# ivargr/kmer_mapper

Hardware: AMD Instinct MI355X
Metric: M k-mers mapped/sec (whole node), k=31 150bp reads (higher is better)
Workload: dtype u64

## Files before the change

### kmer_mapper_amd/csrc/kmm.hip

```cpp
#include <hip/hip_runtime.h>

#include <climits>
#include <cstdarg>
#include <cstdint>
#include <cstdio>
#include <cstdlib>
#include <chrono>
#include <cstring>
#include <memory>
#include <mutex>
#include <string>
#include <thread>
#include <type_traits>
#include <utility>
#include <vector>

#include "kmm.h"
#include "kmm_radix_plan.hpp"

namespace {

thread_local std::string g_err;

int fail(int code, const char *fmt, ...)
// ... 253 lines not shown
    DevPtr<unsigned long long> stats;
    DevPtr<unsigned long long> queue;
    bool dynamic_schedule = true;
    int dyn_chunk = 16;
    uint64_t modulo = 0, magic = 0;
    int64_t n_entries = 0, max_node_id = 0;
    Stage stage[2];
    int cur = 0;
    int n_cu = 256;
    int path = 0;
    int grid_per_cu = 64;
    bool rx_ok = false;
    RxGeometry rx_geo;
    bool rx_no_mid = false;
    bool rx_flush_sorted = true;
    uint32_t rx_max_slice = 0;
    bool rx_fits_small = false, rx_fits_mid = false;
    int rx_grid_per_cu = 2;
    int64_t rx_min_units = 0;
    int64_t rx_sub_cap = RX_SUB_CAP_MAX;
    int64_t rx_sub_cap_eff = 0;
    int rx_sub_cap_eff_age = 0;
    int64_t rx_sub_cap_last = 0;
    const uint32_t *dbg_T1 = nullptr, *dbg_item_base = nullptr;
    const uint16_t *dbg_start1 = nullptr;
    uint32_t dbg_F1 = 0, dbg_NB = 0;
    int host_pack_threads = 0;
    std::unique_ptr<kmm_hostpack::Workers> pack_pool;
    PinnedBuf pack_pinned;
    PinnedBuf ring[RING_SLOTS];
    PinnedBuf pack_bits_pinned;
    int64_t host_packed_calls = 0, host_packed_record_calls = 0;
    int64_t host_pack_slice_kb = 0;
    DevBuf bgzf_comp[2], bgzf_raw[2], bgzf_meta[2], bgzf_tabs, bgzf_err, bgzf_carry, bgzf_crc, bgzf_status;
    Event bgzf_done[2];
    Event bgzf_slot_ev[RING_SLOTS];
    bool bgzf_used[2] = {false, false};
    int bgzf_cur = 0;
    int64_t bgzf_carry_len = 0;
    BgzfStaged bgzf_pre;
    bool bgzf_pre_valid = false;
    const uint8_t *bgzf_pre_from = nullptr, *bgzf_hint_ptr = nullptr;
    int64_t bgzf_pre_n = 0, bgzf_hint_n = 0;
    int bgzf_pre_buf = 0;
    int64_t bgzf_prestaged_calls = 0;
    int64_t bgzf_head_skip = 0;
    int64_t bgzf_tail_stop = -1;
    int64_t bgzf_calls = 0, bgzf_members = 0;
    DevBuf gz_comp, gz_raw, gz_carry, gz_window, gz_tabs, gz_meta, gz_res, gz_win, gz_gmaps, gz_gwin, gz_err;
    std::vector<DevBuf> gz_arena;
    kmm_gunzip::StreamState gz_state;
    int64_t gz_carry_len = 0;
    double gz_ratio = 4.0;
    int64_t gzip_calls = 0, gzip_members = 0, gzip_chunks = 0, gzip_false_starts = 0, gzip_continuations = 0, gzip_inflated = 0;
    int dbg_gzip_chunk_kb = 0;
    DevBuf bam_tiles[2], bam_bad, bam_base, bam_ctl, bam_out;
    int32_t bam_n_ref = -1;
    uint32_t bam_excl = 0;
    int64_t bam_calls = 0, bam_records = 0, bam_excluded = 0, bam_header_bytes = 0, bam_false_starts = 0, bam_continuations = 0;
    DevBuf rs_comp, rs_raw, rs_meta, rs_err, rs_status;
    int64_t bam_n_ref_param = -1;
    int64_t dbg_bam_resync_kb = 0;
    int64_t dbg_bgzf_call_cap_kb = 0;
    int64_t flat_uniform_batches = 0;
    DevBuf sam_tiles, sam_base, sam_ctl;
    int64_t sam_calls = 0, sam_records = 0, sam_excluded = 0, sam_header_lines = 0;
// ... 800 lines not shown
        if (bb >= 4) {
            ix->bloom_words = (uint32_t)(bb / 4);
            occ_bytes = (size_t)ix->bloom_words * 4;
        }
    }
    ix->occ_shift = occ_shift;
    ix->wide = !with_occ;
    if (const char *env = getenv("KMM_WIDE_BUCKETS"))
        ix->wide = atoi(env) != 0;
    HIPCHK(hipMalloc(ix->own_counts_buf.put(), sizeof(uint32_t) * (size_t)(ix->max_node_id + 1)));
    ix->counts = ix->own_counts_buf;
    HIPCHK(hipMemsetAsync(ix->counts, 0, sizeof(uint32_t) * (size_t)(ix->max_node_id + 1), ix->stream));
    HIPCHK(hipMalloc(ix->lut_default.put(), 256));
    HIPCHK(hipMalloc(ix->first_bad.put(), 3 * sizeof(unsigned long long)));
    HIPCHK(hipMalloc(ix->queue.put(), 4 * sizeof(unsigned long long)));
    HIPCHK(hipMalloc(ix->stats.put(), KMM_STAT_BYTES));
    HIPCHK(hipMemset(ix->stats, 0, KMM_STAT_BYTES));
    uint8_t lut[256];
    default_lut(lut);
    HIPCHK(hipMemcpy(ix->lut_default, lut, 256, hipMemcpyHostToDevice));
    HIPCHK(hipMalloc(ix->lut_codes.put(), 256));
    memset(lut, 0xFF, sizeof lut);
    lut[0] = 0; lut[1] = 1; lut[2] = 2; lut[3] = 3;
    HIPCHK(hipMemcpy(ix->lut_codes, lut, 256, hipMemcpyHostToDevice));
    unsigned long long nb[3] = {NO_BAD, NO_BAD, NO_BAD};
    HIPCHK(hipMemcpy(ix->first_bad, nb, sizeof nb, hipMemcpyHostToDevice));
    {
        const int budget = kmm_hostpack::cpu_budget();
        ix->host_pack_threads = budget >= 8 ? (budget < 16 ? budget : 16) : 0;
        if (const char *env = getenv("KMM_HOST_PACK_THREADS")) {
            const int v = atoi(env);
            ix->host_pack_threads = v < 0 ? 0 : (v > 256 ? 256 : v);
        }
    }

    if (ix->host_pack_threads > 0 && (size_t)(ix->max_node_id + 1) * 4 >= ((size_t)64 << 20))
        (void)ensure_ring(ix);

    DevBuf d_h2i, d_nk, d_km, d_nd, d_fr, d_err;
    bool staged = false;
    const int32_t *p_h2i = nullptr, *p_nk = nullptr, *p_nd = nullptr;
    const uint64_t *p_km = nullptr;
    const uint16_t *p_fr = nullptr;
    int rc = KMM_OK;
    do {
        if ((rc = stage_in<int32_t>(ix, d_h2i, h2i, (size_t)M, &p_h2i, &staged))) break;
        if ((rc = stage_in<int32_t>(ix, d_nk, nk, (size_t)M, &p_nk, &staged))) break;
        if ((rc = stage_in<uint64_t>(ix, d_km, kmers, (size_t)N, &p_km, &staged))) break;
        if ((rc = stage_in<int32_t>(ix, d_nd, nodes, (size_t)N, &p_nd, &staged))) break;
        if ((rc = stage_in<uint16_t>(ix, d_fr, freqs, (size_t)N, &p_fr, &staged))) break;
        if ((rc = ensure(d_err, 4))) break;
    } while (0);
    if (rc == KMM_OK) {
        hipError_t e = hipMemsetAsync(d_err.p, 0, 4, ix->copy_stream);
        if (e == hipSuccess) e = hipStreamSynchronize(ix->copy_stream);
        if (e != hipSuccess)
            rc = fail(KMM_ERR_HIP, "index upload: %s", hipGetErrorString(e));
    }
    uint32_t err = 0;
    if (rc == KMM_OK) {
        hipLaunchKernelGGL(k_validate_index, dim3(grid_for(ix, (int64_t)((M + 255) / 256), 16)), dim3(256), 0, ix->stream,
                           p_h2i, p_nk, p_nd, M, N, ix->max_node_id, (uint32_t *)d_err.p);
        hipError_t e = hipGetLastError();
        if (e == hipSuccess) e = hipStreamSynchronize(ix->stream);
        if (e == hipSuccess) e = hipMemcpy(&err, d_err.p, 4, hipMemcpyDeviceToHost);
        if (e != hipSuccess)
// ... 657 lines not shown
        KMMCHK(stage_copies_done(ix));
        HIPCHK(hipMemsetAsync(s.start_bits.p, 0, (size_t)n_words * 4, ix->stream));
        hipLaunchKernelGGL(k_mark_starts, dim3(grid_for(ix, (n_reads + 256) / 256, 8)), dim3(256), 0, ix->stream, d_offs, n_reads,
                           (int64_t)total, (uint32_t *)s.start_bits.p);
        hipLaunchKernelGGL(k_check_offsets, dim3(grid_for(ix, (n_reads + 255) / 256, 8)), dim3(256), 0, ix->stream, d_offs, n_reads,
                           ix->first_bad);
        HIPCHK(hipGetLastError());
        start_bits = (const uint32_t *)s.start_bits.p;
    }
    KMMCHK(rec_launch_flat(ix, (const uint32_t *)s.kmers.p, (int64_t)total, n_reads, start_bits, n_words, read_offsets ? 0 : read_len, k,
                           max_freq, also_revcomp));
    *done = true;
    return stage_release(ix, s, true);
}

static int map_records_host_packed(kmm_index_t *ix, const uint8_t *raw, int64_t n_bytes, int format, int k, int max_freq,
                                   int also_revcomp, int64_t *consumed, int64_t *n_records, bool *done)
{
    *done = false;
    const size_t n = (size_t)n_bytes;
    const size_t code_bytes = (n / 4 + 1024 + 63) & ~(size_t)63, bits_bytes = (n / 8 + 256 + 63) & ~(size_t)63;
    static const bool verbose = getenv("KMM_VERBOSE") != nullptr;
    const auto t_0 = std::chrono::steady_clock::now();
    if (!ensure_pack_pool(ix) || !ensure_pinned(ix->pack_pinned, code_bytes) || !ensure_pinned(ix->pack_bits_pinned, bits_bytes))
        return KMM_OK;
    Stage &s = next_stage(ix);
    KMMCHK(stage_acquire(ix, s));
    KMMCHK(ensure(s.kmers, code_bytes));
    const double ms_alloc = ms_since(t_0);
    const auto t_1 = std::chrono::steady_clock::now();
    kmm_hostpack::RecordsJob job;
    const size_t slice = ix->host_pack_slice_kb > 0 ? (size_t)ix->host_pack_slice_kb << 10 : kmm_hostpack::RecordsJob::slice_bytes();
    job.prepare(raw, n, format == KMM_FORMAT_FASTQ ? 4 : 2, reinterpret_cast<uint64_t *>(ix->pack_pinned.p),
                reinterpret_cast<uint32_t *>(ix->pack_bits_pinned.p), slice);
    ix->pack_pool->start([&job](int) { job.run(); });
    const size_t GROUP = std::max<size_t>(1, ((size_t)32 << 20) / slice);
    int rc = KMM_OK;
    uint64_t copied_w = 0;
    for (size_t g1 = GROUP; g1 < job.n_slices() && rc == KMM_OK; g1 += GROUP) {
        const uint64_t upto_w = job.wait_packed_prefix(g1) >> 5;
        if (upto_w > copied_w) {
            if (hipMemcpyAsync((uint8_t *)s.kmers.p + copied_w * 8, ix->pack_pinned.p + copied_w * 8, (size_t)(upto_w - copied_w) * 8,
                               hipMemcpyHostToDevice, ix->copy_stream) != hipSuccess)
                rc = fail(KMM_ERR_HIP, "hipMemcpyAsync of packed records: %s", hipGetErrorString(hipGetLastError()));
            copied_w = upto_w;
        }
    }
    ix->pack_pool->wait();
    const kmm_hostpack::RecordsResult r = job.finish();
    if (verbose)
        fprintf(stderr, "libkmm: host records packer: %zu bytes, buffers %.2f ms, pack %.2f ms (%.1f GB/s), %d threads, %s\n", n, ms_alloc,
                ms_since(t_1), (double)n / 1e6 / ms_since(t_1), ix->host_pack_threads, r.ok ? "ok" : "refused");
    if (rc != KMM_OK || !r.ok) {
        HIPCHK(hipEventRecord(ix->copied, ix->copy_stream));
        HIPCHK(hipEventSynchronize(ix->copied));
        ix->cur ^= 1;
        return rc;
    }
    ix->map_calls++;
    ix->host_packed_record_calls++;
    if (consumed)
        *consumed = r.consumed;
    if (n_records)
        *n_records = r.n_records;
    *done = true;
    if (r.n_bases <= 0)
        return stage_release(ix, s, copied_w != 0);
    {
        const uint64_t end_w = ((uint64_t)r.n_bases >> 5) + 40, from_w = copied_w < ((uint64_t)r.n_bases >> 5) ? copied_w : ((uint64_t)r.n_bases >> 5);
        HIPCHK(hipMemcpyAsync((uint8_t *)s.kmers.p + from_w * 8, ix->pack_pinned.p + from_w * 8, (size_t)(end_w - from_w) * 8,
                              hipMemcpyHostToDevice, ix->copy_stream));
    }
    const bool uniform = r.uniform_len >= 16;
    const uint32_t *start_bits = nullptr;
    int64_t n_words = 0;
    if (!uniform) {
        n_words = r.n_bases / 32 + 2;
        KMMCHK(ensure(s.start_bits, (size_t)n_words * 4));
        HIPCHK(hipMemcpyAsync(s.start_bits.p, ix->pack_bits_pinned.p, (size_t)n_words * 4, hipMemcpyHostToDevice, ix->copy_stream));
        start_bits = (const uint32_t *)s.start_bits.p;
    }
    KMMCHK(rec_launch_flat(ix, (const uint32_t *)s.kmers.p, r.n_bases, r.n_records, start_bits, n_words, uniform ? r.uniform_len : 0, k,
                           max_freq, also_revcomp));
    return stage_release(ix, s, true);
}
// ... 2483 lines not shown
        if (value && !ix->rx_ok)
            return fail(KMM_ERR_INVALID_ARG, "count_kmers needs the radix path, which is not available for this index");
        KMMCHK(rx_flush(ix));
        HIPCHK(hipStreamSynchronize(ix->stream));
        if (value && !ix->rx_ecnt_acc) {
            const size_t S = ix->rx_S ? ix->rx_S : 1;
            HIPCHK(hipMalloc(ix->rx_ecnt_acc.put(), S * 4));
            HIPCHK(hipMemset(ix->rx_ecnt_acc, 0, S * 4));
        } else if (!value && ix->rx_ecnt_acc) {
            HIPCHK(ix->rx_ecnt_acc.reset());
        }
    } else if (!strcmp(name, "grid_per_cu")) {
        if (value < 1 || value > 1024)
            return fail(KMM_ERR_INVALID_ARG, "grid_per_cu outside [1, 1024]");
        ix->grid_per_cu = (int)value;
    } else if (!strcmp(name, "dynamic_schedule")) {
        ix->dynamic_schedule = value != 0;
    } else if (!strcmp(name, "dyn_chunk")) {
        if (value < 1 || value > 4096)
            return fail(KMM_ERR_INVALID_ARG, "dyn_chunk outside [1, 4096]");
        ix->dyn_chunk = (int)value;
    } else if (!strcmp(name, "occupancy_filter")) {
        ix->use_occ = value != 0;
    } else if (!strcmp(name, "debug_records_copy_stream")) {
        ix->dbg_rec_copy_stream = value != 0;
    } else if (!strcmp(name, "host_pack_threads")) {
        if (value < 0 || value > 256)
            return fail(KMM_ERR_INVALID_ARG, "host_pack_threads outside [0, 256]");
        ix->host_pack_threads = (int)value;
    } else if (!strcmp(name, "host_pack_slice_kb")) {
        if (value < 0 || value > 65536)
            return fail(KMM_ERR_INVALID_ARG, "host_pack_slice_kb outside [0, 65536]");
        ix->host_pack_slice_kb = value;
    } else if (!strcmp(name, "bgzf_head_skip")) {
        if (value < 0)
            return fail(KMM_ERR_INVALID_ARG, "bgzf_head_skip negative");
        ix->bgzf_head_skip = value;
    } else if (!strcmp(name, "bgzf_tail_stop")) {
        ix->bgzf_tail_stop = value < 0 ? -1 : value;
    } else if (!strcmp(name, "debug_bgzf_ring_slot_kb") || !strcmp(name, "debug_ring_slot_kb")) {
        if (value != 0 && (value < 4 || value > (1 << 20) || (value & (value - 1))))
            return fail(KMM_ERR_INVALID_ARG, "debug_ring_slot_kb: 0 or a power of two in [4, 2^20]");
        ix->dbg_bgzf_slot_kb = (int)value;
    } else if (!strcmp(name, "bam_exclude_flags")) {
        if (value < 0 || value > 0xFFFF)
            return fail(KMM_ERR_INVALID_ARG, "bam_exclude_flags outside [0, 0xFFFF]");
        ix->bam_excl = (uint32_t)value;
    } else if (!strcmp(name, "bam_include_flags")) {
        if (value < 0 || value > 0xFFFF)
            return fail(KMM_ERR_INVALID_ARG, "bam_include_flags outside [0, 0xFFFF]");
        ix->bam_incl = (uint32_t)value;
    } else if (!strcmp(name, "bam_min_mapq")) {
        if (value < 0 || value > 255)
            return fail(KMM_ERR_INVALID_ARG, "bam_min_mapq outside [0, 255]");
        ix->bam_min_mapq = (uint32_t)value;
    } else if (!strcmp(name, "bam_n_ref")) {
        if (value < -1 || value > 0x7FFFFFFFll)
            return fail(KMM_ERR_INVALID_ARG, "bam_n_ref outside [-1, 2^31)");
        ix->bam_n_ref_param = value;
    } else if (!strcmp(name, "debug_bam_resync_kb")) {
        if (value < 0 || value > (1ll << 32))
            return fail(KMM_ERR_INVALID_ARG, "debug_bam_resync_kb outside [0, 2^32]");
        ix->dbg_bam_resync_kb = value;
    } else if (!strcmp(name, "debug_bgzf_call_cap_kb")) {
        if (value < 0 || value > (7ll << 19))
            return fail(KMM_ERR_INVALID_ARG, "debug_bgzf_call_cap_kb outside [0, 3.5 GiB / 1 KiB]");
// ... 52 lines not shown
    } else if (!strcmp(name, "debug_records_grid")) {
        if (value < 0 || value > 65536)
            return fail(KMM_ERR_INVALID_ARG, "debug_records_grid outside [0, 65536]");
        ix->dbg_rec_grid = (int)value;
    } else if (!strcmp(name, "debug_skew_p2_counter")) {
        unsigned long long v = 0;
        HIPCHK(hipMemcpy(&v, ix->stats + 2, 8, hipMemcpyDeviceToHost));
        v += (unsigned long long)value;
        HIPCHK(hipMemcpy(ix->stats + 2, &v, 8, hipMemcpyHostToDevice));
        ix->rx_unchecked = true;

    } else {
        return fail(KMM_ERR_INVALID_ARG, "unknown parameter '%s'", name);
    }
    return KMM_OK;
}

int kmm_get_param(kmm_index_t *ix, const char *name, int64_t *value)
{
    if (!ix || !name || !value)
        return fail(KMM_ERR_INVALID_ARG, "NULL argument");
    if (!strcmp(name, "path"))
        *value = ix->path;
    else if (!strcmp(name, "part_shift"))
        *value = ix->rx_geo.w;
    else if (!strcmp(name, "radix_min_units"))
        *value = ix->rx_min_units;
    else if (!strcmp(name, "radix_grid_per_cu"))
        *value = ix->rx_grid_per_cu;
    else if (!strcmp(name, "host_pack_threads"))
        *value = ix->host_pack_threads;
    else if (!strcmp(name, "host_pack_slice_kb"))
        *value = ix->host_pack_slice_kb;
    else if (!strcmp(name, "host_packed_calls"))
        *value = ix->host_packed_calls;
    else if (!strcmp(name, "host_packed_record_calls"))
        *value = ix->host_packed_record_calls;
    else if (!strcmp(name, "bgzf_prestaged_calls"))
        *value = ix->bgzf_prestaged_calls;
    else if (!strcmp(name, "gzip_calls"))
        *value = ix->gzip_calls;
    else if (!strcmp(name, "gzip_members"))
        *value = ix->gzip_members;
    else if (!strcmp(name, "gzip_chunks"))
        *value = ix->gzip_chunks;
    else if (!strcmp(name, "gzip_false_starts"))
        *value = ix->gzip_false_starts;
    else if (!strcmp(name, "gzip_continuations"))
        *value = ix->gzip_continuations;
    else if (!strcmp(name, "gzip_inflated_bytes"))
        *value = ix->gzip_inflated;
    else if (!strcmp(name, "debug_gzip_chunk_kb"))
        *value = ix->dbg_gzip_chunk_kb;
    else if (!strcmp(name, "min_base_quality"))
        *value = ix->min_base_quality;
    else if (!strcmp(name, "use_record_qual"))
        *value = ix->use_record_qual;
    else if (!strcmp(name, "original_strand"))
        *value = ix->original_strand;
    else if (!strcmp(name, "debug_records_piece_kb"))
        *value = ix->dbg_rec_piece_kb;
    else if (!strcmp(name, "debug_records_grid"))
        *value = ix->dbg_rec_grid;
    else if (!strcmp(name, "record_hits"))
        *value = ix->record_hits;
    else if (!strcmp(name, "record_hits_pending"))
// ... 177 lines not shown
```

### kmer_mapper_amd/csrc/kmm_hostpack.hpp

```cpp
#pragma once

#include <sched.h>
#include <unistd.h>

#include <algorithm>
#include <atomic>
#include <chrono>
#include <condition_variable>
#include <cstdint>
#include <cstdio>
#include <cstdlib>
#include <cstring>
#include <functional>
#include <mutex>
#include <thread>
#include <vector>

#if defined(__x86_64__)
#include <immintrin.h>
#endif

namespace kmm_hostpack {

inline int cpu_budget()
{
    int n = 0;
    cpu_set_t set;
    CPU_ZERO(&set);
    if (sched_getaffinity(0, sizeof set, &set) == 0)
        n = CPU_COUNT(&set);
    if (n < 1)
        n = (int)sysconf(_SC_NPROCESSORS_ONLN);
    long long quota = -1, period = 0;
    if (FILE *f = fopen("/sys/fs/cgroup/cpu.max", "r")) {
        char q[64] = {0};
        if (fscanf(f, "%63s %lld", q, &period) == 2 && strcmp(q, "max") != 0)
            quota = atoll(q);
        fclose(f);
    } else if (FILE *g = fopen("/sys/fs/cgroup/cpu/cpu.cfs_quota_us", "r")) {
        if (fscanf(g, "%lld", &quota) != 1)
            quota = -1;
        fclose(g);
        if (FILE *p = fopen("/sys/fs/cgroup/cpu/cpu.cfs_period_us", "r")) {
            if (fscanf(p, "%lld", &period) != 1)
                period = 0;
            fclose(p);
// ... 352 lines not shown
        prepare(s, n_bases, d, chunk_bases);
        const int nt = (size_t)n_threads < n_chunks ? n_threads : (int)n_chunks;
        for (int t = 0; t < nt; ++t)
            threads.emplace_back([this] { run(); });
    }
    void join()
    {
        for (auto &t : threads)
            t.join();
        threads.clear();
    }
    ~Job() { join(); }
};

struct RecordsResult {
    bool ok = false;
    int64_t consumed = 0;
    int64_t n_records = 0;
    int64_t n_bases = 0;
    int64_t uniform_len = 0;
};

class RecordsJob {
  public:
    static size_t slice_bytes()
    {
        static const size_t v = [] {
            const char *env = getenv("KMM_HOST_PACK_SLICE_KB");
            const long kb = env ? atol(env) : 1024;
            return (size_t)(kb < 4 ? 4 : (kb > 65536 ? 65536 : kb)) << 10;
        }();
        return v;
    }
    static long spin_us()
    {
        static const long v = [] {
            const char *env = getenv("KMM_HOST_PACK_SPIN_US");
            return env ? atol(env) : 300L;
        }();
        return v;
    }

    void prepare(const uint8_t *raw, size_t n, int period, uint64_t *codes, uint32_t *start_bits, size_t slice = 0)
    {
        raw_ = raw;
        n_ = n;
        pm_ = (uint32_t)period - 1u;
        hc_ = period == 4 ? (uint8_t)'@' : (uint8_t)'>';
        codes_ = codes;
        bits_ = start_bits;
        SLICE = slice ? (slice < 4096 ? 4096 : slice) : slice_bytes();
        n_slices_ = (n + SLICE - 1) / SLICE;
        desc_ = std::vector<Desc>(n_slices_ + 1);
        desc_[0].line = 0;
        desc_[0].flat = 0;
        desc_[0].ready.store(1, std::memory_order_release);
        next_.store(0);
        watch_ = 0;
        abort_.store(false);
        bad_struct_.store(~0ull);
        bad_base_.store(~0ull);
        n_marks_.store(0);
        n_off_.store(0);
        lguess_ = 0;
        const uint8_t *a = n ? (const uint8_t *)memchr(raw, '\n', n) : nullptr;
        if (a) {
            const uint8_t *b = (const uint8_t *)memchr(a + 1, '\n', n - (size_t)(a + 1 - raw));
            if (b) {
                size_t len = (size_t)(b - (a + 1));
                if (len && b[-1] == '\r')
                    --len;
                lguess_ = len;
            }
        }
    }

    void run()
    {
        std::vector<uint32_t> nlbuf(SLICE + 1);
        for (;;) {
            const size_t i = next_.fetch_add(1);
            if (i >= n_slices_)
                return;
            if (abort_.load(std::memory_order_relaxed)) {
                desc_[i + 1].ready.store(1, std::memory_order_release);
                desc_[i].packed.store(1, std::memory_order_release);
                continue;
            }
            const size_t b0 = i * SLICE, b1 = b0 + SLICE < n_ ? b0 + SLICE : n_;
            Census c;
            c.nlpos = nlbuf.data();
            census(raw_ + b0, b1 - b0, c);
            if (!desc_[i].ready.load(std::memory_order_acquire)) {
                const auto t_wait = std::chrono::steady_clock::now();
                unsigned spins = 0;
                while (!desc_[i].ready.load(std::memory_order_acquire)) {
                    cpu_relax();
                    if ((++spins & 255u) == 0 &&
                        std::chrono::steady_clock::now() - t_wait > std::chrono::microseconds(spin_us()))
                        std::this_thread::sleep_for(std::chrono::microseconds(50));
                }
            }
            const uint64_t line0 = desc_[i].line, flat0 = desc_[i].flat;
            uint64_t seq = 0;
            for (uint32_t r = 0; r < 4u; ++r)
                if (((line0 + r) & pm_) == 1u)
                    seq += c.by_phase[r];
            const uint64_t flat1 = flat0 + seq;
            if ((flat1 & 31u) && (flat1 & ~(uint64_t)31) >= flat0) {
                codes_[flat1 >> 5] = 0;
                bits_[flat1 >> 5] = 0;
            }
            desc_[i + 1].line = line0 + c.n_nl;
            desc_[i + 1].flat = flat1;
            desc_[i + 1].ready.store(1, std::memory_order_release);
            pack_slice(b0, b1, c.nlpos, c.n_nl, line0, flat0, flat1, c.has_cr);
        }
    }

    RecordsResult finish()
    {
        RecordsResult r;
        if (abort_.load())
            return r;
        const uint64_t total_lines = desc_[n_slices_].line, flat_total = desc_[n_slices_].flat;
        const uint64_t period = (uint64_t)pm_ + 1u, target = total_lines - total_lines % period;
        size_t cut = 0;
        if (target) {
            uint64_t skip = total_lines - target;
            size_t p = n_;
            for (;;) {
                while (p > 0 && raw_[p - 1] != '\n')
                    --p;
                if (skip == 0)
                    break;
                --skip;
                --p;
            }
            cut = p;
        }
        uint64_t tail_seq = 0;
        {
            size_t p = cut;
            while (p < n_ && raw_[p] != '\n')
                ++p;
            if (p < n_) {
                ++p;
                while (p < n_ && raw_[p] != '\n') {
                    if (raw_[p] != '\r')
                        ++tail_seq;
                    ++p;
// ... 23 lines not shown
            bits_[w + 1] = bits_[w + 2] = 0;
        }
        r.ok = true;
        r.consumed = (int64_t)cut;
        r.n_records = (int64_t)(target / period);
        r.n_bases = (int64_t)flat_end;
        const uint64_t marks = n_marks_.load() - tail_marks;
        if (lguess_ >= 1 && r.n_records > 0 && n_off_.load() == 0 && marks == (uint64_t)r.n_records && tail_marks <= 1 &&
            flat_end == (uint64_t)r.n_records * lguess_)
            r.uniform_len = (int64_t)lguess_;
        return r;
    }

    size_t n_slices() const { return n_slices_; }

    uint64_t wait_packed_prefix(size_t upto)
    {
        if (upto > n_slices_)
            upto = n_slices_;
        while (watch_ < upto) {
            if (desc_[watch_].packed.load(std::memory_order_acquire))
                ++watch_;
            else
                std::this_thread::sleep_for(std::chrono::microseconds(40));
        }
        return desc_[upto].flat;
    }

  private:
    struct alignas(64) Desc {
        std::atomic<uint32_t> ready{0};
        std::atomic<uint32_t> packed{0};
        uint64_t line = 0, flat = 0;
        Desc() = default;
        Desc(const Desc &o) : ready(o.ready.load()), packed(o.packed.load()), line(o.line), flat(o.flat) {}
    };

    static inline void cpu_relax()
    {
#if defined(__x86_64__)
        _mm_pause();
#endif
    }

    struct Census {
        uint32_t *nlpos;
        size_t n_nl = 0;
        uint64_t by_phase[4] = {0, 0, 0, 0};
        uint32_t r = 0;
        size_t run = 0;
        bool has_cr = false;
    };

    static inline void census_events(Census &c, size_t base, uint64_t m_nl, uint64_t m_cr)
    {
        if (__builtin_expect(m_cr != 0, 0)) {
            uint64_t m = m_nl | m_cr;
            uint32_t r = c.r;
            while (m) {
                const unsigned b = (unsigned)__builtin_ctzll(m);
                m &= m - 1;
                if ((m_nl >> b) & 1u)
                    r = (r + 1u) & 3u;
                else
                    c.by_phase[r] -= 1;
            }
            c.has_cr = true;
        }
        while (m_nl) {
// ... 35 lines not shown
        }
        return q;
    }
    __attribute__((target("avx2"))) static size_t census_avx2(const uint8_t *p, size_t len, Census &c)
    {
        const __m256i nl = _mm256_set1_epi8('\n'), cr = _mm256_set1_epi8('\r');
        size_t q = 0;
        for (; q + 64 <= len; q += 64) {
            const __m256i a = _mm256_loadu_si256(reinterpret_cast<const __m256i *>(p + q));
            const __m256i b = _mm256_loadu_si256(reinterpret_cast<const __m256i *>(p + q + 32));
            const uint64_t m_nl = (uint32_t)_mm256_movemask_epi8(_mm256_cmpeq_epi8(a, nl)) |
                                  ((uint64_t)(uint32_t)_mm256_movemask_epi8(_mm256_cmpeq_epi8(b, nl)) << 32);
            const uint64_t m_cr = (uint32_t)_mm256_movemask_epi8(_mm256_cmpeq_epi8(a, cr)) |
                                  ((uint64_t)(uint32_t)_mm256_movemask_epi8(_mm256_cmpeq_epi8(b, cr)) << 32);
            if (m_nl | m_cr)
                census_events(c, q, m_nl, m_cr);
        }
        return q;
    }
#endif

    static void census(const uint8_t *p, size_t len, Census &c)
    {
        size_t q = 0;
#if defined(__x86_64__)
        const Isa l = isa();
        if (l == ISA_AVX512)
            q = census_avx512(p, len, c);
        else if (l == ISA_AVX2)
            q = census_avx2(p, len, c);
#endif
        census_scalar(p, len, q, c);
        c.by_phase[c.r] += len - c.run;
    }

    struct Writer {
        uint64_t *out;
        uint64_t acc = 0;
        unsigned fill;
        uint64_t *shared;
        inline void store_word()
        {
            if (out == shared)
                __atomic_fetch_or(out, acc, __ATOMIC_RELAXED);
            else
                *out = acc;
            ++out;
        }
        inline void push(uint64_t w, unsigned nb)
        {
            acc |= w << fill;
            if (fill + nb >= 64u) {
                store_word();
                acc = fill ? w >> (64u - fill) : 0ull;
                fill = fill + nb - 64u;
            } else {
                fill += nb;
            }
        }
        inline void flush()
        {
            if (fill)
                __atomic_fetch_or(out, acc, __ATOMIC_RELAXED);
        }
    };

// ... 78 lines not shown
    inline void emit_run(PackState &s, const uint8_t *p, size_t len)
    {
        if (!len)
            return;
        if (s.pending)
            mark(s);
#if defined(__x86_64__)
        if (isa() == ISA_AVX512)
            emit_avx512(s, p, len);
        else
#endif
            emit_scalar(s, p, len);
        s.flat += len;
    }

    inline void emit_seq(PackState &s, const uint8_t *p, size_t len, bool may_have_cr, bool ends_line)
    {
        if (may_have_cr) {
            if (ends_line && len && p[len - 1] == '\r')
                --len;
            while (len) {
                const uint8_t *c = (const uint8_t *)memchr(p, '\r', len);
                if (!c)
                    break;
                emit_run(s, p, (size_t)(c - p));
                s.pending = true;
                len -= (size_t)(c - p) + 1;
                p = c + 1;
            }
        }
        emit_run(s, p, len);
    }

    void pack_slice(size_t b0, size_t b1, const uint32_t *nlpos, size_t n_nl, uint64_t line0, uint64_t flat0, uint64_t flat1, bool has_cr)
    {
        PackState s;
        s.w.out = codes_ + (flat0 >> 5);
        s.w.fill = (unsigned)(2u * (flat0 & 31u));
        s.w.shared = s.w.fill ? s.w.out : nullptr;
        s.flat = flat0;
        s.next_mult = lguess_ ? (flat0 + lguess_ - 1) / lguess_ * lguess_ : 0;
        {
            const uint64_t w0 = (flat0 + 31) >> 5, w1 = flat1 >> 5;
            if (w1 > w0) {
                memset(bits_ + w0, 0, (size_t)(w1 - w0) * 4);
                s.own0 = w0;
                s.own1 = w1;
            }
        }
        const uint8_t *base = raw_ + b0;
        const size_t len = b1 - b0;
        bool at_line_start = b0 == 0 || raw_[b0 - 1] == '\n';
        s.pending = !at_line_start && ((line0 & pm_) == 1u) && raw_[b0 - 1] == '\r';
        uint64_t bad_struct = ~0ull;
        size_t pos = 0;
        uint64_t line = line0;
        for (size_t k = 0; k <= n_nl; ++k) {
            const size_t end = k < n_nl ? nlpos[k] : len;
            const uint32_t phase = (uint32_t)line & pm_;
            if (phase == 1u) {
                if (at_line_start)
                    s.pending = true;
                emit_seq(s, base + pos, end - pos, has_cr, k < n_nl);
            } else if (at_line_start && pos < len && !(phase & 1u)) {
                const uint8_t want = phase == 0u ? hc_ : (uint8_t)'+';
                if (base[pos] != want && bad_struct == ~0ull)
                    bad_struct = b0 + pos;
            }
            if (k < n_nl) {
                pos = end + 1;
                ++line;
                at_line_start = true;
            }
        }
        s.w.flush();
        desc_[(b0 / SLICE)].packed.store(1, std::memory_order_release);
        if (s.marks)
            n_marks_.fetch_add(s.marks, std::memory_order_relaxed);
        if (s.off)
            n_off_.fetch_add(s.off, std::memory_order_relaxed);
        if (bad_struct != ~0ull)
            atomic_min(bad_struct_, bad_struct);
        if (s.bad)
            atomic_min(bad_base_, (uint64_t)b0);
        (void)flat1;
    }

    static void atomic_min(std::atomic<uint64_t> &a, uint64_t v)
    {
        uint64_t cur = a.load(std::memory_order_relaxed);
        while (v < cur && !a.compare_exchange_weak(cur, v, std::memory_order_relaxed)) {
        }
    }

    const uint8_t *raw_ = nullptr;
    size_t SLICE = (size_t)256 << 10;
    size_t n_ = 0, n_slices_ = 0;
    uint32_t pm_ = 3;
    uint8_t hc_ = '@';
    uint64_t *codes_ = nullptr;
    uint32_t *bits_ = nullptr;
    uint64_t lguess_ = 0;
    std::vector<Desc> desc_;
    std::atomic<size_t> next_{0};
    size_t watch_ = 0;
    std::atomic<bool> abort_{false};
    std::atomic<uint64_t> bad_struct_{~0ull}, bad_base_{~0ull}, n_marks_{0}, n_off_{0};
};

}
```

Before: 178,600.

## Add one-pass speculative FASTQ walk to host record packer, skipping census pass

For FASTQ on AVX-512 hosts, each slice worker now guesses a record start, walks and packs records speculatively into scratch in a single pass, then shifts the packed words into place once the predecessor's offset is known. This removes the separate census pass (newline scan) that previously had to run before packing, and lets slices whose records were already consumed by a predecessor's tail be skipped. It adds AVX-512 prefetch, non-temporal shifted copies, and a fallback to the census path when the guess or walk fails. It also increases code complexity and scratch memory per thread.

```diff
diff --git a/kmer_mapper_amd/csrc/kmm.hip b/kmer_mapper_amd/csrc/kmm.hip
--- a/kmer_mapper_amd/csrc/kmm.hip
+++ b/kmer_mapper_amd/csrc/kmm.hip
@@ -309,6 +309,8 @@
     PinnedBuf pack_bits_pinned;
     int64_t host_packed_calls = 0, host_packed_record_calls = 0;
     int64_t host_pack_slice_kb = 0;
+    bool host_pack_one_pass = true;
+    int64_t host_pack_one_pass_slices = 0, host_pack_census_slices = 0;
     DevBuf bgzf_comp[2], bgzf_raw[2], bgzf_meta[2], bgzf_tabs, bgzf_err, bgzf_carry, bgzf_crc, bgzf_status;
     Event bgzf_done[2];
     Event bgzf_slot_ev[RING_SLOTS];
@@ -1175,6 +1177,7 @@
             const int v = atoi(env);
             ix->host_pack_threads = v < 0 ? 0 : (v > 256 ? 256 : v);
         }
+        ix->host_pack_one_pass = kmm_hostpack::RecordsJob::one_pass_default();
     }
 
     if (ix->host_pack_threads > 0 && (size_t)(ix->max_node_id + 1) * 4 >= ((size_t)64 << 20))
@@ -1898,7 +1901,7 @@
     kmm_hostpack::RecordsJob job;
     const size_t slice = ix->host_pack_slice_kb > 0 ? (size_t)ix->host_pack_slice_kb << 10 : kmm_hostpack::RecordsJob::slice_bytes();
     job.prepare(raw, n, format == KMM_FORMAT_FASTQ ? 4 : 2, reinterpret_cast<uint64_t *>(ix->pack_pinned.p),
-                reinterpret_cast<uint32_t *>(ix->pack_bits_pinned.p), slice);
+                reinterpret_cast<uint32_t *>(ix->pack_bits_pinned.p), slice, ix->host_pack_one_pass ? 1 : 0);
     ix->pack_pool->start([&job](int) { job.run(); });
     const size_t GROUP = std::max<size_t>(1, ((size_t)32 << 20) / slice);
     int rc = KMM_OK;
@@ -1914,9 +1917,12 @@
     }
     ix->pack_pool->wait();
     const kmm_hostpack::RecordsResult r = job.finish();
+    ix->host_pack_one_pass_slices += (int64_t)job.one_pass_slices();
+    ix->host_pack_census_slices += (int64_t)job.census_slices();
     if (verbose)
-        fprintf(stderr, "libkmm: host records packer: %zu bytes, buffers %.2f ms, pack %.2f ms (%.1f GB/s), %d threads, %s\n", n, ms_alloc,
-                ms_since(t_1), (double)n / 1e6 / ms_since(t_1), ix->host_pack_threads, r.ok ? "ok" : "refused");
+        fprintf(stderr, "libkmm: host records packer: %zu bytes, buffers %.2f ms, pack %.2f ms (%.1f GB/s), %d threads, slices %llu one-pass + %llu census, %s\n",
+                n, ms_alloc, ms_since(t_1), (double)n / 1e6 / ms_since(t_1), ix->host_pack_threads, (unsigned long long)job.one_pass_slices(),
+                (unsigned long long)job.census_slices(), r.ok ? "ok" : "refused");
     if (rc != KMM_OK || !r.ok) {
         HIPCHK(hipEventRecord(ix->copied, ix->copy_stream));
         HIPCHK(hipEventSynchronize(ix->copied));
@@ -4466,6 +4472,8 @@
         if (value < 0 || value > 65536)
             return fail(KMM_ERR_INVALID_ARG, "host_pack_slice_kb outside [0, 65536]");
         ix->host_pack_slice_kb = value;
+    } else if (!strcmp(name, "host_pack_one_pass")) {
+        ix->host_pack_one_pass = value != 0;
     } else if (!strcmp(name, "bgzf_head_skip")) {
         if (value < 0)
             return fail(KMM_ERR_INVALID_ARG, "bgzf_head_skip negative");
@@ -4584,6 +4592,12 @@
         *value = ix->host_pack_threads;
     else if (!strcmp(name, "host_pack_slice_kb"))
         *value = ix->host_pack_slice_kb;
+    else if (!strcmp(name, "host_pack_one_pass"))
+        *value = ix->host_pack_one_pass ? 1 : 0;
+    else if (!strcmp(name, "host_pack_one_pass_slices"))
+        *value = ix->host_pack_one_pass_slices;
+    else if (!strcmp(name, "host_pack_census_slices"))
+        *value = ix->host_pack_census_slices;
     else if (!strcmp(name, "host_packed_calls"))
         *value = ix->host_packed_calls;
     else if (!strcmp(name, "host_packed_record_calls"))
diff --git a/kmer_mapper_amd/csrc/kmm_hostpack.hpp b/kmer_mapper_amd/csrc/kmm_hostpack.hpp
--- a/kmer_mapper_amd/csrc/kmm_hostpack.hpp
+++ b/kmer_mapper_amd/csrc/kmm_hostpack.hpp
@@ -12,6 +12,7 @@
 #include <cstdlib>
 #include <cstring>
 #include <functional>
+#include <memory>
 #include <mutex>
 #include <thread>
 #include <vector>
@@ -430,6 +431,23 @@
         }();
         return v;
     }
+    static bool one_pass_default()
+    {
+        static const bool v = [] {
+            const char *env = getenv("KMM_HOST_PACK_ONE_PASS");
+            return env ? atoi(env) != 0 : true;
+        }();
+        return v;
+    }
+    static size_t prefetch_bytes()
+    {
+        static const size_t v = [] {
+            const char *env = getenv("KMM_HOST_PACK_PREFETCH");
+            const long b = env ? atol(env) : 2048;
+            return (size_t)(b < 0 ? 0 : (b > 65536 ? 65536 : b));
+        }();
+        return v;
+    }
     static long spin_us()
     {
         static const long v = [] {
@@ -439,8 +457,11 @@
         return v;
     }
 
-    void prepare(const uint8_t *raw, size_t n, int period, uint64_t *codes, uint32_t *start_bits, size_t slice = 0)
-    {
+    void prepare(const uint8_t *raw, size_t n, int period, uint64_t *codes, uint32_t *start_bits, size_t slice = 0, int one_pass = -1)
+    {
+        one_pass_ = period == 4 && isa() == ISA_AVX512 && (one_pass < 0 ? one_pass_default() : one_pass != 0);
+        n_one_pass_.store(0);
+        n_census_.store(0);
         raw_ = raw;
         n_ = n;
         pm_ = (uint32_t)period - 1u;
@@ -452,6 +473,7 @@
         desc_ = std::vector<Desc>(n_slices_ + 1);
         desc_[0].line = 0;
         desc_[0].flat = 0;
+        desc_[0].end = 0;
         desc_[0].ready.store(1, std::memory_order_release);
         next_.store(0);
         watch_ = 0;
@@ -475,7 +497,7 @@
 
     void run()
     {
-        std::vector<uint32_t> nlbuf(SLICE + 1);
+        Scratch sc;
         for (;;) {
             const size_t i = next_.fetch_add(1);
             if (i >= n_slices_)
@@ -486,9 +508,24 @@
                 continue;
             }
             const size_t b0 = i * SLICE, b1 = b0 + SLICE < n_ ? b0 + SLICE : n_;
+            Walk wk;
+            bool guessed = false;
+#if defined(__x86_64__)
+            if (one_pass_) {
+                const size_t s = guess_start(i, b0, b1);
+                if (s != NONE) {
+                    guessed = true;
+                    walk(s, b1, sc, wk);
+                }
+            }
+#endif
             Census c;
-            c.nlpos = nlbuf.data();
-            census(raw_ + b0, b1 - b0, c);
+            bool have_census = false;
+            if (!one_pass_ || (guessed && wk.status == WALK_GAVE_UP)) {
+                c.nlpos = sc.nl(SLICE);
+                census(raw_ + b0, b1 - b0, c);
+                have_census = true;
+            }
             if (!desc_[i].ready.load(std::memory_order_acquire)) {
                 const auto t_wait = std::chrono::steady_clock::now();
                 unsigned spins = 0;
@@ -500,21 +537,35 @@
                 }
             }
             const uint64_t line0 = desc_[i].line, flat0 = desc_[i].flat;
-            uint64_t seq = 0;
-            for (uint32_t r = 0; r < 4u; ++r)
-                if (((line0 + r) & pm_) == 1u)
-                    seq += c.by_phase[r];
-            const uint64_t flat1 = flat0 + seq;
-            if ((flat1 & 31u) && (flat1 & ~(uint64_t)31) >= flat0) {
-                codes_[flat1 >> 5] = 0;
-                bits_[flat1 >> 5] = 0;
-            }
-            desc_[i + 1].line = line0 + c.n_nl;
-            desc_[i + 1].flat = flat1;
-            desc_[i + 1].ready.store(1, std::memory_order_release);
-            pack_slice(b0, b1, c.nlpos, c.n_nl, line0, flat0, flat1, c.has_cr);
-        }
-    }
+            const size_t end0 = desc_[i].end;
+            if (end0 >= b1) {
+                publish(i, line0, flat0, end0);
+                desc_[i].packed.store(1, std::memory_order_release);
+                n_one_pass_.fetch_add(1, std::memory_order_relaxed);
+                continue;
+            }
+            if (wk.status != WALK_GAVE_UP && wk.start == end0 && (line0 & 3u) == 0u) {
+                commit_walk(i, wk, sc, line0, flat0);
+                n_one_pass_.fetch_add(1, std::memory_order_relaxed);
+                continue;
+            }
+            if (!have_census || end0 != b0) {
+                c = Census();
+                c.nlpos = sc.nl(SLICE);
+                census(raw_ + end0, b1 - end0, c);
+            }
+            const uint64_t flat1 = flat0 + seq_bytes(c, line0);
+            zero_shared_word(flat0, flat1);
+            publish(i, line0 + c.n_nl, flat1, b1);
+            if (pack_slice(end0, b1, c.nlpos, c.n_nl, line0, flat0, flat1, c.has_cr))
+                atomic_min(bad_base_, (uint64_t)b0);
+            desc_[i].packed.store(1, std::memory_order_release);
+            n_census_.fetch_add(1, std::memory_order_relaxed);
+        }
+    }
+
+    uint64_t one_pass_slices() const { return n_one_pass_.load(); }
+    uint64_t census_slices() const { return n_census_.load(); }
 
     RecordsResult finish()
     {
@@ -604,9 +655,75 @@
         std::atomic<uint32_t> ready{0};
         std::atomic<uint32_t> packed{0};
         uint64_t line = 0, flat = 0;
+        size_t end = 0;
         Desc() = default;
-        Desc(const Desc &o) : ready(o.ready.load()), packed(o.packed.load()), line(o.line), flat(o.flat) {}
+        Desc(const Desc &o) : ready(o.ready.load()), packed(o.packed.load()), line(o.line), flat(o.flat), end(o.end) {}
     };
+
+    inline void publish(size_t i, uint64_t line, uint64_t flat, size_t end)
+    {
+        desc_[i + 1].line = line;
+        desc_[i + 1].flat = flat;
+        desc_[i + 1].end = end;
+        desc_[i + 1].ready.store(1, std::memory_order_release);
+    }
+    inline void zero_shared_word(uint64_t flat0, uint64_t flat1)
+    {
+        if ((flat1 & 31u) && (flat1 & ~(uint64_t)31) >= flat0) {
+            codes_[flat1 >> 5] = 0;
+            bits_[flat1 >> 5] = 0;
+        }
+    }
+
+    struct Scratch {
+        std::unique_ptr<uint32_t[]> nlbuf;
+        std::unique_ptr<uint64_t[]> words;
+        size_t cap = 0;
+        std::unique_ptr<uint32_t[]> starts;
+        uint32_t *nl(size_t slice)
+        {
+            if (!nlbuf)
+                nlbuf.reset(new uint32_t[slice + 1]);
+            return nlbuf.get();
+        }
+    };
+
+    static constexpr size_t NONE = ~(size_t)0;
+    enum { WALK_GAVE_UP = 0, WALK_OK = 1, WALK_OK_TAIL = 2 };
+    struct Walk {
+        int status = WALK_GAVE_UP;
+        size_t start = 0, end = 0;
+        uint64_t n_rec = 0, n_bases = 0;
+    };
+
+    size_t guess_start(size_t i, size_t b0, size_t b1) const
+    {
+        if (i == 0)
+            return 0;
+        size_t p = b0;
+        if (raw_[b0 - 1] != '\n') {
+            const uint8_t *e = (const uint8_t *)memchr(raw_ + b0, '\n', n_ - b0);
+            if (!e)
+                return NONE;
+            p = (size_t)(e - raw_) + 1;
+        }
+        for (int tries = 0; tries < 5 && p < b1; ++tries) {
+            const uint8_t *l1 = (const uint8_t *)memchr(raw_ + p, '\n', n_ - p);
+            if (!l1)
+                return NONE;
+            const size_t a = (size_t)(l1 - raw_) + 1;
+            if (raw_[p] == '@') {
+                const uint8_t *l2 = a < n_ ? (const uint8_t *)memchr(raw_ + a, '\n', n_ - a) : nullptr;
+                if (!l2)
+                    return NONE;
+                if ((size_t)(l2 - raw_) + 1 < n_ && l2[1] == '+')
+                    return p;
+            }
+            p = a;
+        }
+        return NONE;
+    }
+
 
     static inline void cpu_relax()
     {
@@ -708,6 +825,15 @@
 #endif
         census_scalar(p, len, q, c);
         c.by_phase[c.r] += len - c.run;
+    }
+
+    inline uint64_t seq_bytes(const Census &c, uint64_t line0) const
+    {
+        uint64_t seq = 0;
+        for (uint32_t r = 0; r < 4u; ++r)
+            if (((line0 + r) & pm_) == 1u)
+                seq += c.by_phase[r];
+        return seq;
     }
 
     struct Writer {
@@ -852,7 +978,7 @@
         emit_run(s, p, len);
     }
 
-    void pack_slice(size_t b0, size_t b1, const uint32_t *nlpos, size_t n_nl, uint64_t line0, uint64_t flat0, uint64_t flat1, bool has_cr)
+    bool pack_slice(size_t b0, size_t b1, const uint32_t *nlpos, size_t n_nl, uint64_t line0, uint64_t flat0, uint64_t flat1, bool has_cr)
     {
         PackState s;
         s.w.out = codes_ + (flat0 >> 5);
@@ -894,16 +1020,309 @@
             }
         }
         s.w.flush();
-        desc_[(b0 / SLICE)].packed.store(1, std::memory_order_release);
         if (s.marks)
             n_marks_.fetch_add(s.marks, std::memory_order_relaxed);
         if (s.off)
             n_off_.fetch_add(s.off, std::memory_order_relaxed);
         if (bad_struct != ~0ull)
             atomic_min(bad_struct_, bad_struct);
-        if (s.bad)
-            atomic_min(bad_base_, (uint64_t)b0);
-        (void)flat1;
+        return s.bad;
+    }
+
+#if defined(__x86_64__)
+    KMM_AVX512_TARGET static inline size_t find_nl(const uint8_t *raw, size_t from, size_t n)
+    {
+        const __m512i nl = _mm512_set1_epi8('\n');
+        size_t q = from;
+        for (; q + 64 <= n; q += 64) {
+            const uint64_t m = _mm512_cmpeq_epi8_mask(_mm512_loadu_si512(raw + q), nl);
+            if (m)
+                return q + (unsigned)__builtin_ctzll(m);
+        }
+        if (q < n) {
+            const __mmask64 live = ~0ull >> (64 - (n - q));
+            const uint64_t m = _mm512_mask_cmpeq_epi8_mask(live, _mm512_maskz_loadu_epi8(live, raw + q), nl);
+            if (m)
+                return q + (unsigned)__builtin_ctzll(m);
+        }
+        return n;
+    }
+    KMM_AVX512_TARGET static inline bool has_nl(const uint8_t *raw, size_t from, size_t len)
+    {
+        const __m512i nl = _mm512_set1_epi8('\n');
+        uint64_t m = 0;
+        size_t q = 0;
+        for (; q + 64 <= len; q += 64)
+            m |= _mm512_cmpeq_epi8_mask(_mm512_loadu_si512(raw + from + q), nl);
+        if (q < len) {
+            const __mmask64 live = ~0ull >> (64 - (len - q));
+            m |= _mm512_mask_cmpeq_epi8_mask(live, _mm512_maskz_loadu_epi8(live, raw + from + q), nl);
+        }
+        return m != 0;
+    }
+
+    KMM_AVX512_TARGET void walk(size_t s, size_t b1, Scratch &sc, Walk &wk) const
+    {
+        const uint8_t *raw = raw_;
+        const size_t n = n_;
+        if (!sc.words) {
+            sc.cap = SLICE / 32 + 64;
+            sc.words.reset(new uint64_t[sc.cap]);
+            sc.starts.reset(new uint32_t[SLICE / 8 + 2]);
+        }
+        const __m512i t0 = _mm512_load_si512(tab128().t), t1 = _mm512_load_si512(tab128().t + 64);
+        const __m512i nlv = _mm512_set1_epi8('\n');
+        __m512i flags = _mm512_setzero_si512();
+        uint64_t bad = 0;
+        uint64_t *out = sc.words.get(), *cap_end = out + sc.cap;
+        uint64_t acc = 0;
+        unsigned fill = 0;
+        uint32_t *starts = sc.starts.get();
+        uint64_t n_rec = 0, n_bases = 0;
+        size_t p = s, pf = s;
+        const size_t ahead = prefetch_bytes();
+        int tail = 0;
+        wk.start = s;
+#define KMM_WALK_PUSH64(word)                                                                                                         \
+    do {                                                                                                                              \
+        const uint64_t w_ = (word);                                                                                                   \
+        *out++ = acc | (w_ << fill);                                                                                                  \
+        acc = (w_ >> 1) >> (63u - fill);                                                                                              \
+    } while (0)
+#define KMM_WALK_PUSH(word, nbits)                                                                                                    \
+    do {                                                                                                                              \
+        const uint64_t w_ = (word);                                                                                                   \
+        const unsigned tot_ = fill + (nbits);                                                                                         \
+        const uint64_t full_ = acc | (w_ << fill), over_ = (w_ >> 1) >> (63u - fill);                                                 \
+        *out = full_;                                                                                                                 \
+        out += tot_ >> 6;                                                                                                             \
+        acc = tot_ >= 64u ? over_ : full_;                                                                                            \
+        fill = tot_ & 63u;                                                                                                            \
+    } while (0)
+        while (p < b1) {
+            const size_t rec_word = (size_t)(out - sc.words.get());
+            const uint64_t rec_acc = acc;
+            const unsigned rec_fill = fill;
+            if (raw[p] != '@')
+                return;
+            for (const size_t want = p + ahead < n ? p + ahead : n; pf < want; pf += 64)
+                _mm_prefetch(reinterpret_cast<const char *>(raw + pf), _MM_HINT_T0);
+            const size_t h = find_nl(raw, p + 1, n);
+            if (h == n) {
+                tail = 1;
+                break;
+            }
+            const size_t a = h + 1;
+            size_t len = 0;
+            for (;;) {
+                if (out + 4 > cap_end) {
+                    const size_t used = (size_t)(out - sc.words.get());
+                    std::unique_ptr<uint64_t[]> grown(new uint64_t[sc.cap * 2]);
+                    memcpy(grown.get(), sc.words.get(), used * 8);
+                    sc.words = std::move(grown);
+                    sc.cap *= 2;
+                    out = sc.words.get() + used;
+                    cap_end = sc.words.get() + sc.cap;
+                }
+                const size_t pos = a + len;
+                __m512i v;
+                uint64_t m;
+                if (pos + 64 <= n) {
+                    v = _mm512_loadu_si512(raw + pos);
+                    m = _mm512_cmpeq_epi8_mask(v, nlv);
+                    if (!m) {
+                        const __m128i o = codes64_avx512(v, t0, t1, flags);
+                        KMM_WALK_PUSH64((uint64_t)_mm_cvtsi128_si64(o));
+                        KMM_WALK_PUSH64((uint64_t)_mm_extract_epi64(o, 1));
+                        len += 64;
+                        continue;
+                    }
+                } else {
+                    if (pos == n) {
+                        tail = 1;
+                        break;
+                    }
+                    const __mmask64 live = ~0ull >> (64 - (n - pos));
+                    v = _mm512_maskz_loadu_epi8(live, raw + pos);
+                    m = _mm512_mask_cmpeq_epi8_mask(live, v, nlv);
+                    if (!m) {
+                        tail = 1;
+                        break;
+                    }
+                }
+                const unsigned k = (unsigned)__builtin_ctzll(m);
+                if (k) {
+                    const __mmask64 lv = ~0ull >> (64 - k);
+                    __m512i f2 = _mm512_setzero_si512();
+                    const __m128i o = codes64_avx512(_mm512_maskz_mov_epi8(lv, v), t0, t1, f2);
+                    bad |= _mm512_movepi8_mask(f2) & lv;
+                    if (k <= 32) {
+                        KMM_WALK_PUSH((uint64_t)_mm_cvtsi128_si64(o), 2u * k);
+                    } else {
+                        KMM_WALK_PUSH64((uint64_t)_mm_cvtsi128_si64(o));
+                        KMM_WALK_PUSH((uint64_t)_mm_extract_epi64(o, 1), 2u * (k - 32u));
+                    }
+                }
+                len += k;
+                break;
+            }
+            if (!tail) {
+                if (len == 0)
+                    return;
+                const size_t c = a + len + 1;
+                size_t q = 0;
+                if (c >= n) {
+                    tail = 1;
+                } else if (raw[c] != '+') {
+                    return;
+                } else if (c + 1 < n && raw[c + 1] == '\n') {
+                    q = c + 2;
+                } else {
+                    const size_t e = find_nl(raw, c + 1, n);
+                    if (e == n)
+                        tail = 1;
+                    else
+                        q = e + 1;
+                }
+                if (!tail) {
+                    if (q + len >= n) {
+                        if (has_nl(raw, q, n - q))
+                            return;
+                        tail = 1;
+                    } else if (raw[q + len] != '\n' || has_nl(raw, q, len)) {
+                        return;
+                    }
+                }
+                if (!tail) {
+                    if (n_bases > 0x7fffffffull)
+                        return;
+                    starts[n_rec++] = (uint32_t)n_bases;
+                    n_bases += len;
+                    p = q + len + 1;
+                    continue;
+                }
+            }
+            out = sc.words.get() + rec_word;
+            acc = rec_acc;
+            fill = rec_fill;
+            break;
+        }
+#undef KMM_WALK_PUSH
+#undef KMM_WALK_PUSH64
+        if (_mm512_movepi8_mask(flags) | bad)
+            return;
+        if (tail && n - p > 0x7fffffffull)
+            return;
+        if (fill)
+            *out = acc;
+        wk.status = tail ? WALK_OK_TAIL : WALK_OK;
+        wk.end = p;
+        wk.n_rec = n_rec;
+        wk.n_bases = n_bases;
+    }
+#endif
+
+#if defined(__x86_64__)
+    KMM_AVX512_TARGET static void shift_copy_avx512(uint64_t *dst, const uint64_t *src, uint64_t j0, uint64_t j1, unsigned sh)
+    {
+        const __m128i up = _mm_cvtsi32_si128((int)sh), down = _mm_cvtsi32_si128((int)(64u - sh));
+        for (uint64_t j = j0; j < j1; j += 8) {
+            const __m512i v = _mm512_loadu_si512(src + j), prev = _mm512_loadu_si512(src + j - 1);
+            const __m512i w = _mm512_or_si512(_mm512_sll_epi64(v, up), _mm512_srl_epi64(prev, down));
+            _mm512_stream_si512(reinterpret_cast<__m512i *>(dst + j), w);
+        }
+    }
+#endif
+
+    void commit_walk(size_t i, const Walk &wk, Scratch &sc, uint64_t line0, uint64_t flat0)
+    {
+        const uint64_t flat_a = flat0 + wk.n_bases, line_a = line0 + 4u * wk.n_rec;
+        uint64_t flat1 = flat_a, line1 = line_a;
+        size_t end1 = wk.end;
+        Census c;
+        if (wk.status == WALK_OK_TAIL) {
+            c.nlpos = sc.nl(SLICE);
+            census(raw_ + wk.end, n_ - wk.end, c);
+            flat1 = flat_a + seq_bytes(c, line_a);
+            line1 = line_a + c.n_nl;
+            end1 = n_;
+            zero_shared_word(flat0, flat_a);
+        }
+        zero_shared_word(flat0, flat1);
+        publish(i, line1, flat1, end1);
+        const uint64_t own0 = (flat0 + 31) >> 5, own1 = flat_a >> 5;
+        if (own1 > own0)
+            memset(bits_ + own0, 0, (size_t)(own1 - own0) * 4);
+        uint64_t off = 0, next_mult = lguess_ ? (flat0 + lguess_ - 1) / lguess_ * lguess_ : 0;
+        const uint32_t *starts = sc.starts.get();
+        for (uint64_t r = 0; r < wk.n_rec; ++r) {
+            const uint64_t f = flat0 + starts[r], wi = f >> 5;
+            if (wi >= own0 && wi < own1)
+                bits_[wi] |= 1u << (f & 31u);
+            else
+                __atomic_fetch_or(&bits_[wi], 1u << (f & 31u), __ATOMIC_RELAXED);
+            if (lguess_) {
+                if (f == next_mult) {
+                    next_mult += lguess_;
+                } else {
+                    const uint64_t rem = f % lguess_;
+                    if (rem)
+                        ++off;
+                    next_mult = f - rem + lguess_;
+                }
+            }
+        }
+        if (wk.n_bases) {
+            uint64_t *dst = codes_ + (flat0 >> 5);
+            const unsigned sh = (unsigned)(2u * (flat0 & 31u));
+            const uint64_t *src = sc.words.get();
+            const uint64_t bits = 2u * wk.n_bases, n_src = (bits + 63u) >> 6, n_dst = (sh + bits + 63u) >> 6;
+            const bool last_shared = ((sh + bits) & 63u) != 0;
+            uint64_t carry = 0;
+            for (uint64_t j = 0; j < n_dst; ++j) {
+#if defined(__x86_64__)
+                if (j >= 1 && j + 8 < n_dst && j + 8 <= n_src && (reinterpret_cast<uintptr_t>(dst + j) & 63u) == 0) {
+                    const uint64_t j1 = j + ((n_src < n_dst - 1 ? n_src : n_dst - 1) - j) / 8 * 8;
+                    shift_copy_avx512(dst, src, j, j1, sh);
+                    carry = (src[j1 - 1] >> 1) >> (63u - sh);
+                    j = j1 - 1;
+                    continue;
+                }
+#endif
+                const uint64_t v = j < n_src ? src[j] : 0ull;
+                const uint64_t word = (v << sh) | carry;
+                carry = (v >> 1) >> (63u - sh);
+                if ((j == 0 && sh) || (j + 1 == n_dst && last_shared)) {
+                    __atomic_fetch_or(dst + j, word, __ATOMIC_RELAXED);
+                } else {
+#if defined(__x86_64__)
+                    _mm_stream_si64(reinterpret_cast<long long *>(dst + j), (long long)word);
+#else
+                    dst[j] = word;
+#endif
+                }
+            }
+#if defined(__x86_64__)
+            _mm_sfence();
+#endif
+        }
+        if (wk.n_rec)
+            n_marks_.fetch_add(wk.n_rec, std::memory_order_relaxed);
+        if (off)
+            n_off_.fetch_add(off, std::memory_order_relaxed);
+        if (wk.status == WALK_OK_TAIL) {
+            if (pack_slice(wk.end, n_, c.nlpos, c.n_nl, line_a, flat_a, flat1, c.has_cr)) {
+                const uint8_t *t = code_tab().t;
+                size_t x = wk.end;
+                while (x < n_ && raw_[x] != '\n')
+                    ++x;
+                for (++x; x < n_ && raw_[x] != '\n'; ++x)
+                    if (raw_[x] != '\r' && (t[raw_[x]] & 0x80u))
+                        break;
+                atomic_min(bad_base_, (uint64_t)((x < n_ ? x : n_ - 1) / SLICE * SLICE));
+            }
+        }
+        desc_[i].packed.store(1, std::memory_order_release);
     }
 
     static void atomic_min(std::atomic<uint64_t> &a, uint64_t v)
@@ -926,6 +1345,8 @@
     size_t watch_ = 0;
     std::atomic<bool> abort_{false};
     std::atomic<uint64_t> bad_struct_{~0ull}, bad_base_{~0ull}, n_marks_{0}, n_off_{0};
+    bool one_pass_ = false;
+    std::atomic<uint64_t> n_one_pass_{0}, n_census_{0};
 };
 
 }
```

Result: slower. 176,500 (-1.2%).
